# TomClabault/SYCL-ray-tracing

Measured on AMD Instinct MI355X. Metric: Msamples/sec (W×H×spp/s) at 1080p; per-channel L∞ vs CPU ref, higher is better.
Workload: dtype f32; 1 GPU; cfg2: PBRT Dragon stand-in (1,000,002 tris) 1920x1080x64spp x8 bounces, SKY-L 2048x1024 env IS+MIS; W=1920, H=1080, spp=64, bounces=8, parallelism=1 GPU

## Files before the change

sycl-ray-tracing_amd/csrc/rt_render.hip:

```cpp
#include <hip/hip_runtime.h>

#include "rt_backend_hip.h"
#include "rt_wave.h"
#include "rt_wave_kernels.h"
#include "rt_quad.h"
#include "rt_row.h"
#include "rt_octet.h"

namespace {

#if RT_DEBUG_FB
__device__ unsigned long long rt_dbg_fb[8];
#define RT_DBG(i) atomicAdd(&rt_dbg_fb[i], 1ull)
#else
#define RT_DBG(i) ((void)0)
#endif
__device__ __forceinline__ int lane_id() { return __lane_id(); }

template <int N>
struct LdsStack {
    static constexpr int CAP = N;
    uint32_t* r;
    float* k;
    __device__ __forceinline__ uint32_t rec(int i) const { return r[i * 256]; }
    __device__ __forceinline__ float key(int i) const { return k[i * 256]; }
    __device__ __forceinline__ void set(int i, uint32_t rv, float kv)
    {
        r[i * 256] = rv;
        k[i * 256] = kv;
    }
    __device__ __forceinline__ void set_rec(int i, uint32_t rv) { r[i * 256] = rv; }
};

__device__ __forceinline__ int wave_gid() { return (int)((blockIdx.x * blockDim.x + threadIdx.x) >> 6); }
__device__ __forceinline__ int wave_count() { return (int)((gridDim.x * blockDim.x) >> 6); }

template <bool STATS>
__device__ __forceinline__ void flush_stats(const rtk::Stats& st, unsigned long long* out)
{
    if (STATS)
        for (int i = 0; i < RT_STAT_COUNT; i++)
            if (st.c[i]) atomicAdd(&out[i], st.c[i]);
}

__host__ __device__ __forceinline__ size_t qbase(bool heavy, int shard, size_t seg_cap)
{
    return heavy ? ((size_t)RT_QSHARDS + (size_t)shard * (RT_QSHARDS / RT_HSHARDS)) * seg_cap : (size_t)shard * seg_cap;
}

template <class E>
__device__ __forceinline__ void append_emit(const rtk::WaveView& W, int pout, int base, int n_in, int p, const E& e)
{
    const int cps = ((n_in + 63) / 64 + RT_QSHARDS - 1) / RT_QSHARDS;
    const int sh = min(RT_QSHARDS - 1, (base >> 6) / cps);
    const size_t seg = (size_t)sh * W.seg_cap;
    const unsigned long long lt = (lane_id() == 0) ? 0ull : (~0ull >> (64 - lane_id()));
    if (W.r_heavy) {
        const int hs = sh % RT_HSHARDS;
        unsigned long long b[2 * rtk::RK_COUNT + 1];
#pragma unroll
        for (int k = 0; k < rtk::RK_COUNT; k++) {
            const bool m = (e.mask >> k) & 1u;
            b[k] = __ballot(m && !e.heavy);
            b[rtk::RK_COUNT + k] = __ballot(m && e.heavy);
        }
        b[2 * rtk::RK_COUNT] = __ballot(e.active);
        int r[2 * rtk::RK_COUNT + 1];
        if (lane_id() == 0) {
#pragma unroll
            for (int k = 0; k <= 2 * rtk::RK_COUNT; k++) {
                const int c = k < rtk::RK_COUNT ? qc_at(pout, k, sh)
                              : k < 2 * rtk::RK_COUNT ? hc_at(pout, k - rtk::RK_COUNT, hs)
                                                      : ac_at(pout, sh);
                r[k] = b[k] ? atomicAdd(W.counters + c, __popcll(b[k])) : 0;
            }
        }
#pragma unroll
        for (int k = 0; k < rtk::RK_COUNT; k++) {
            const int ih = __shfl(r[rtk::RK_COUNT + k], 0) + __popcll(b[rtk::RK_COUNT + k] & lt);
            const int i = __shfl(r[k], 0) + __popcll(b[k] & lt);
            if ((e.mask >> k) & 1u) W.q[k][e.heavy ? qbase(true, hs, W.seg_cap) + ih : qbase(false, sh, W.seg_cap) + i] = e.rec(k, p);
        }
        const int a = __shfl(r[2 * rtk::RK_COUNT], 0) + __popcll(b[2 * rtk::RK_COUNT] & lt);
        if (e.active) W.act_out[seg + a] = p;
        return;
    }
    unsigned long long b[rtk::RK_COUNT + 1];
#pragma unroll
    for (int k = 0; k < rtk::RK_COUNT; k++) b[k] = __ballot((e.mask >> k) & 1u);
    b[rtk::RK_COUNT] = __ballot(e.active);
    int r[rtk::RK_COUNT + 1];
    if (lane_id() == 0) {
#pragma unroll
        for (int k = 0; k <= rtk::RK_COUNT; k++)
            r[k] = b[k] ? atomicAdd(W.counters + (k < rtk::RK_COUNT ? qc_at(pout, k, sh) : ac_at(pout, sh)),
                                    __popcll(b[k]))
                        : 0;
    }
#pragma unroll
    for (int k = 0; k < rtk::RK_COUNT; k++) {
        const int i = __shfl(r[k], 0) + __popcll(b[k] & lt);
        if ((e.mask >> k) & 1u) W.q[k][qbase(false, sh, W.seg_cap) + i] = e.rec(k, p);
    }
    const int a = __shfl(r[rtk::RK_COUNT], 0) + __popcll(b[rtk::RK_COUNT] & lt);
    if (e.active) W.act_out[seg + a] = p;
}


template <class AT>
__device__ __forceinline__ void shard_prefix(const int32_t* cnt, int m, AT at, int* pre)
{
    const int nw = (int)(blockDim.x >> 6), w = (int)(threadIdx.x >> 6);
    for (int g = w; g < m / 64; g += nw) {
        int v = cnt[at(g * 64 + lane_id())];
        for (int o = 1; o < 64; o <<= 1) {
            const int u = __shfl_up(v, o);
            if (lane_id() >= o) v += u;
        }
        pre[g * 64 + lane_id() + 1] = v;
    }
    __syncthreads();
    int add[8];
    const int ng = m / 64;
    for (int g = w; g < ng && g < 8 * nw; g += nw) {
        int off = 0;
        for (int h = 0; h < g; h++) off += pre[h * 64 + 64];
        add[g / nw] = off;
    }
    __syncthreads();
    for (int g = w; g < ng && g < 8 * nw; g += nw) pre[g * 64 + lane_id() + 1] += add[g / nw];
    if (threadIdx.x == 0) pre[0] = 0;
    __syncthreads();
}

template <int M>
__device__ __forceinline__ int shard_find8(const int* pre, int g)
{
    constexpr int TOP = M > 512 ? 512 : M > 64 ? 64 : M > 8 ? 8 : 1;
    static_assert(M <= 4096, "three or four 8-way rounds");
    int lo = 0;
#pragma unroll
    for (int step = TOP; step >= 1; step >>= 3) {
        int c = 0;
#pragma unroll
        for (int k = 1; k < 8; k++) {
            const int j = lo + step * k;
            c += (j < M && pre[j] <= g) ? 1 : 0;
        }
        lo += step * c;
    }
    return lo;
}

__device__ __forceinline__ const rtk::RayRec* queue_item_ptr(const rtk::WaveView& W, const int* pre, int g, int& kind)
{
    const int j = shard_find8<RT_NSEG>(pre, g);
    const SegId s = seg_id(j);
    kind = s.kind;
    rtk::RayRec* qk = W.q[0];
#pragma unroll
    for (int k2 = 1; k2 < rtk::RK_COUNT; k2++) qk = s.kind == k2 ? W.q[k2] : qk;
    return qk + qbase(s.heavy, s.shard, W.seg_cap) + (g - pre[j]);
}

struct QPrefetch {
    float4_* buf;
    int* kind;
};
__device__ __forceinline__ void queue_prefetch(const rtk::WaveView& W, const int* pre, const QPrefetch& pf, int first, int cursor,
                                               int wg, int wn, int total)
{
    const int lane = lane_id(), i = lane >> 1;
    const int j = cursor + i;
    const int idx = (wg + (j >> 4) * wn) * 16 + (j & 15);
    const bool ok = lane < 32 && idx < total;
    int kind = -1;
    if (ok) {
        const rtk::RayRec* rp = queue_item_ptr(W, pre, first + idx, kind);
        __builtin_amdgcn_global_load_lds((const void*)((const float4_*)rp + (lane & 1)),
                                         (__attribute__((address_space(3))) void*)pf.buf, 16, 0, 0);
    }
    if (lane < 32 && (lane & 1) == 0) pf.kind[i] = ok ? kind : -1;
}

__global__ __launch_bounds__(256) void k_init(rtk::WaveView W)
{
    rtlibm::lds_tables_init();
    const int p = blockIdx.x * blockDim.x + threadIdx.x;
    rtk::Emit e;
    e.mask = 0;
    e.active = false;
    e.heavy = false;
    if (p < W.n_slots) rtk::path_init(W, p, e);
    append_emit(W, 0, p & ~63, W.n_slots, p, e);
}

__global__ __launch_bounds__(256) void k_resume(rtk::WaveView W)
{
    rtlibm::lds_tables_init();
    const int p = blockIdx.x * blockDim.x + threadIdx.x;
    rtk::Emit e;
    e.mask = 0;
    e.active = false;
    e.heavy = false;
    if (p < W.n_slots) rtk::path_resume(W, p, e);
    append_emit(W, 0, p & ~63, W.n_slots, p, e);
}

__global__ __launch_bounds__(256) void k_resolve(const float4_* __restrict__ base, const float4_* __restrict__ state,
                                                 float4_* __restrict__ out, int n, int done)
{
    rtlibm::lds_tables_init();
    const int i = blockIdx.x * blockDim.x + threadIdx.x;
    if (i < n) out[i] = rtk::resolve_pixel(base[i], state[i], done);
}

__global__ __launch_bounds__(256) void k_tonemap(rtk::WaveView W)
{
    rtlibm::lds_tables_init();
    const int p = blockIdx.x * blockDim.x + threadIdx.x;
    if (p < W.n_slots) rtk::tonemap_pixel(W, p);
}

#define RT_LDS_WORDS 16
#define RT_REFILL 16
#ifndef RT_TRACE_REFILL
#define RT_TRACE_REFILL 4
#endif

__device__ __forceinline__ bool forced_fallback(const rtk::WaveView& W, const float4_& o, const float4_& d)
{
    return (W.far_check && rtk::far_origin(W.S, rtk::v3of(o))) || rtk::forced_fallback(W.force_fb, o, d);
}

__device__ __forceinline__ int split_blocks(int nb, int w0, int w1)
{
    if (w0 + w1 == 0) return 0;
    int n0 = (int)((long)nb * w0 / ((long)w0 + w1));
    if (w0 > 0 && n0 == 0) n0 = 1;
    if (w1 > 0 && n0 == nb) n0 = nb - 1;
    return n0;
}

__device__ __forceinline__ void walk_done(const rtk::WaveView& W, int par, uint32_t target)
{
    const int j = atomicAdd(W.counters + C_DONE0 + par, 1);
    W.done[par][j] = (int32_t)(target >> 3);
}

template <bool ANY>
__device__ void exact_octets(const rtk::WaveView& W, int par, uint32_t* lds, int lane, int n_res, int total,
                             rtk::Stats* st)
{
    rtk::OctRing w = rtk::oct_ring(lds);
    const int sub = lane_id() & 7;
    uint32_t* spr = W.spill_r + (size_t)(lane & ~7) * RT_STACK_CAP;
    float* spk = W.spill_k + (size_t)(lane & ~7) * RT_STACK_CAP;
    const rtk::RayRec* fb = ANY ? W.fb_a[par] : W.fb_c[par];
    int32_t* ticket = W.counters + (ANY ? C_TK_EXACT_A : C_TK_EXACT_C);
    int32_t* parked = W.counters + (ANY ? C_PARKA0 : C_PARKC0) + par;
    rtk::TravG T;
    bool has = false, drained = false;
    uint32_t target = 0;
    auto done = [&]() {
        if (sub == 0) {
            if (ANY)
                rtk::finish_any(W, target, T.hit);
            else
                rtk::finish_closest(W, target, T.o, T.d, T.best_t, T.best_k);
            walk_done(W, par, target);
        }
    };
    for (;;) {
        const unsigned long long bneed = __ballot(!has && sub == 0);
        const int nneed = __popcll(bneed);
        if (!drained && (nneed >= RT_REFILL / 8 || nneed == 8)) {
            int base = 0;
            if (lane_id() == 0) base = atomicAdd(ticket, nneed);
            base = __shfl(base, 0);
            if (base + nneed >= total) drained = true;
            if (!has) {
                const int idx = base + __popcll(bneed & ((1ull << rtk::oct_lane0()) - 1ull));
                if (idx < n_res) {
                    target = ANY ? rtk::octa_resume(W.S, &W.park_a[par ^ 1][idx], T, w, sub)
                                 : rtk::octc_resume(W.S, &W.park_c[par ^ 1][idx], T, w, sub);
                    has = true;
                } else if (idx < total) {
                    const rtk::RayRec r = fb[idx - n_res];
                    target = (rt_asuint(r.o.w) << 3) | rt_asuint(r.d.w);
                    if (st && sub == 0) st->c[RT_STAT_FALLBACK]++;
                    has = rtk::octg_setup(W.S, T, rtk::v3of(r.o), rtk::v3of(r.d), st, ANY, sub);
                    if (!has) done();
                }
            }
        }
        if (!__any(has)) {
            if (drained) break;
            continue;
        }
        if (has) {
            if (ANY)
                rtk::octa_node(W.S, T, w, spr, sub, st);
            else
                rtk::octc_node(W.S, T, w, spr, spk, sub, st);
            if (T.mode == rtk::TM_DONE) {
                done();
                has = false;
            } else if (T.steps >= W.budget && (ANY ? rtk::octa_parkable(T) : rtk::octc_parkable(T))) {
                int ps = 0;
                if (sub == 0) ps = atomicAdd(parked, 1);
                if (sub == 0) RT_DBG(1);
                ps = __shfl(ps, rtk::oct_lane0());
                if (ps < W.park_cap) {
                    if (ANY)
                        rtk::octa_park(T, w, target, &W.park_a[par][ps], sub);
                    else
                        rtk::octc_park(T, w, target, &W.park_c[par][ps], sub);
                    has = false;
                } else {
                    T.steps = 0;
                }
            }
        }
    }
}

template <bool STATS, bool PROG = false>
__global__ __launch_bounds__(256) __attribute__((amdgpu_waves_per_eu(RT_STEP_OCC, 8))) void k_step(rtk::WaveView W, int par, unsigned long long* stats)
{
    __shared__ uint32_t s_lds[6 * rtk::RK_COUNT * 256];
    static_assert(6 * rtk::RK_COUNT >= RT_LDS_WORDS, "the exact roles' stacks fit the emit columns");
    __shared__ int s_pre[RT_QSHARDS + 1];
    rtlibm::lds_tables_init();
    rtk::lds_shade_init(W.S);
    int32_t* cnt = W.counters;
    if (blockIdx.x == 0 && threadIdx.x == 0) {
        cnt[C_FBC0 + (par ^ 1)] = cnt[C_FBA0 + (par ^ 1)] = 0;
        cnt[C_DONE0 + (par ^ 1)] = 0;
        const int nf = cnt[C_FBC0 + par] + cnt[C_FBA0 + par];
        if (W.handovers && nf > 0) atomicAdd(W.handovers, (unsigned long long)nf);
    }
    rtk::Stats st;
    if (STATS)
        for (int i = 0; i < RT_STAT_COUNT; i++) st.c[i] = 0;
    rtk::Stats* ps = STATS ? &st : nullptr;
    const int nrc = min(cnt[C_PARKC0 + (par ^ 1)], W.park_cap), nra = min(cnt[C_PARKA0 + (par ^ 1)], W.park_cap);
    const int ec = nrc + cnt[C_FBC0 + par], ea = nra + cnt[C_FBA0 + par];
    const int half = min(W.spill_lanes / 512, max(1, (int)gridDim.x / 4));
    constexpr int WPB = 32;
    const int nbe_c = min(half, (ec + WPB - 1) / WPB), nbe_a = min(half, (ea + WPB - 1) / WPB);
    const int b = (int)blockIdx.x;
    if (b < nbe_c) {
        exact_octets<false>(W, par, s_lds, b * 256 + (int)threadIdx.x, nrc, ec, ps);
        flush_stats<STATS>(st, stats);
        return;
    }
    if (b < nbe_c + nbe_a) {
        exact_octets<true>(W, par, s_lds, (W.spill_lanes / 512 + b - nbe_c) * 256 + (int)threadIdx.x, nra, ea, ps);
        flush_stats<STATS>(st, stats);
        return;
    }
    shard_prefix(cnt, RT_QSHARDS, [&](int j) { return ac_at(par, j); }, s_pre);
    const int n = s_pre[RT_QSHARDS];
    if (STATS && W.iterq && b == nbe_c + nbe_a && threadIdx.x == 0 && W.iter < RT_MAX_TIMED_ITERS)
        W.iterq[2 * W.iter + 1] = n;
    const int nbs = (int)gridDim.x - (nbe_c + nbe_a);
    const int wg = (b - nbe_c - nbe_a) * (int)(blockDim.x >> 6) + (int)(threadIdx.x >> 6);
    const int wn = nbs * (int)(blockDim.x >> 6);
    for (int base = wg * 64; base < n; base += wn * 64) {
        const int idx = base + lane_id();
        rtk::EmitLds<256> e;
        e.s = reinterpret_cast<float*>(s_lds) + threadIdx.x;
        e.mask = 0;
        e.active = false;
        e.heavy = false;
        int p = -1;
        if (idx < n) {
            const int sh = shard_find8<RT_QSHARDS>(s_pre, idx);
            p = W.act_in[(size_t)sh * W.seg_cap + (idx - s_pre[sh])];
            rtk::path_step<PROG>(W, p, e, ps);
        }
        append_emit(W, par ^ 1, base, n, p, e);
    }
    flush_stats<STATS>(st, stats);
}

__global__ __launch_bounds__(256) void k_hand(rtk::WaveView W, int par)
{
    __shared__ int s_pre[RT_QSHARDS + 1];
    shard_prefix(W.counters, RT_QSHARDS, [&](int j) { return ac_at(par, j); }, s_pre);
    const int n = s_pre[RT_QSHARDS];
    for (int idx = (int)(blockIdx.x * blockDim.x + threadIdx.x); idx < n; idx += (int)(gridDim.x * blockDim.x)) {
        const int sh = shard_find8<RT_QSHARDS>(s_pre, idx);
        const int p = W.act_in[(size_t)sh * W.seg_cap + (idx - s_pre[sh])];
        if ((int)rt_asuint(W.p_thr[p].w) > W.fast_thr || W.r_park[p] != 0) continue;
        const int j = atomicAdd(W.fast_ticket, 1);
        if (j >= W.fast_cap) continue;
        W.fast_list[j] = p;
        W.r_park[p] = -1;
    }
}

__global__ __launch_bounds__(256) void k_hist(rtk::WaveView W, int par, int32_t* __restrict__ hist)
{
    __shared__ int s_pre[RT_QSHARDS + 1];
    shard_prefix(W.counters, RT_QSHARDS, [&](int j) { return ac_at(par, j); }, s_pre);
    const int n = s_pre[RT_QSHARDS];
    for (int idx = (int)(blockIdx.x * blockDim.x + threadIdx.x); idx < n; idx += (int)(gridDim.x * blockDim.x)) {
        const int sh = shard_find8<RT_QSHARDS>(s_pre, idx);
        const int p = W.act_in[(size_t)sh * W.seg_cap + (idx - s_pre[sh])];
        atomicAdd(hist + min((int)rt_asuint(W.p_thr[p].w), W.spp), 1);
    }
}

__device__ __noinline__ void walk_log(const rtk::WaveView& W, rtk::V3 o, rtk::V3 d, uint32_t target, int calls, float t,
                                      int k, int where)
{
    if (W.wlog_every < 0 && t != -2.0f) return;
    if (W.wlog_every > 1 && ((target * 2654435761u) ^ ((uint32_t)W.iter * 40503u)) % (uint32_t)W.wlog_every != 0u) return;
    const int i = atomicAdd(W.wlog_n, 1);
    if (i >= W.wlog_cap) return;
    float4_* r = W.wlog + 3 * (size_t)i;
    r[0] = float4_{o.x, o.y, o.z, rt_asfloat((target & 7u) | ((uint32_t)where << 8))};
    r[1] = float4_{d.x, d.y, d.z, rt_asfloat((uint32_t)calls)};
    r[2] = float4_{t, rt_asfloat((uint32_t)k), rt_asfloat((uint32_t)W.iter), rt_asfloat(target >> 3)};
}

struct RowInQuadStack {
    static constexpr int CAP = 4 * RT_QSTACK;
    uint32_t* r;
    float* k;
    __device__ __forceinline__ uint32_t rec(int i) const { return r[(i >> 2) * 64 + (i & 3)]; }
    __device__ __forceinline__ float key(int i) const { return k[(i >> 2) * 64 + (i & 3)]; }
    __device__ __forceinline__ void set(int i, uint32_t rv, float kv)
    {
        r[(i >> 2) * 64 + (i & 3)] = rv;
        k[(i >> 2) * 64 + (i & 3)] = kv;
    }
    __device__ __forceinline__ void set_rec(int i, uint32_t rv) { r[(i >> 2) * 64 + (i & 3)] = rv; }
};

#if RT_DRAIN_STRONG_FENCE
#define RT_DRAIN_FENCE()                                       \
    do {                                                       \
        __builtin_amdgcn_fence(__ATOMIC_SEQ_CST, "workgroup"); \
        __builtin_amdgcn_s_waitcnt(0);                         \
        __builtin_amdgcn_wave_barrier();                       \
    } while (0)
#else
#define RT_DRAIN_FENCE()                                       \
    do {                                                       \
        __builtin_amdgcn_fence(__ATOMIC_ACQ_REL, "wavefront"); \
        __builtin_amdgcn_wave_barrier();                       \
    } while (0)
#endif

template <bool ANY, bool STATS, bool PAIR, int G, int BRUTE, class QSTK>
__device__ __forceinline__ void trace_stream(const rtk::WaveView& W, const RtSceneView& S, QSTK& stk, const int* s_pre,
                                             int first, int total, int wg, int wn, int32_t* fbn, rtk::RayRec* fbl,
                                             rtk::Stats* ps, const QPrefetch& pf)
{
    static_assert(G == 4 || G == 16, "quads or rows");
    constexpr int REFILL = G == 4 ? RT_TRACE_REFILL : 1;
    const int lane = lane_id(), qd = lane / G;
    int sub = lane & (G - 1);
    int cursor = 0;
    bool exhausted = wg * 16 >= total;
    bool active = false;
    uint32_t target = 0;
    rtk::QState q;
    if (!exhausted) queue_prefetch(W, s_pre, pf, first, cursor, wg, wn, total);
    auto finish = [&](int res, int gs) {
        if (W.r_heavy && sub == 0 && q.calls >= W.heavy_calls) W.r_heavy[target >> 3] = 1;
        if (STATS && W.iterq && sub == 0 && W.iter < RT_MAX_TIMED_ITERS) {
            int32_t* q2 = W.iterq + 2 * RT_MAX_TIMED_ITERS + 4 * W.iter;
            atomicMax(q2 + (ANY ? 1 : 0), q.calls);
            if (q.calls > 8) atomicAdd(q2 + 2, 1);
        }
        float t = 0.0f;
        int k = 0;
        int why = res < 0 ? 3 : 0;
        if (res > 0 && !ANY && !rtk::quad_closest_answer<BRUTE>(S, q, sub & 3, t, k, gs == 4 || sub == 0 ? ps : nullptr)) {
            res = -1;
            why = q.h.tie ? 1 : 2;
        }
        if (STATS && W.wlog && sub == 0 && q.calls >= W.wlog_min)
            walk_log(W, q.o, q.d, target, q.calls, res <= 0 ? -2.0f : ANY ? (float)(q.h.k == 1) : t, res <= 0 ? why : k,
                     gs == 4 ? 0 : 1);
        if (sub == 0) {
            if (res > 0) {
                if (ANY)
                    rtk::finish_any(W, target, q.h.k == 1);
                else
                    rtk::finish_closest(W, target, q.o, q.d, t, k);
            } else {
                fbl[atomicAdd(fbn, 1)] = rtk::RayRec{rtk::f4(q.o, rt_asfloat(target >> 3)),
                                                     rtk::f4(q.d, rt_asfloat(target & 7u))};
                RT_DBG(ANY ? 2 : 0);
                RT_DBG(why == 3 ? 3 : why == 1 ? 4 : 5);
                if (gs == 16) RT_DBG(6);
                atomicAdd(&W.r_park[target >> 3], 1);
                if (STATS && W.iterq && W.iter < RT_MAX_TIMED_ITERS)
                    atomicAdd(W.iterq + 2 * RT_MAX_TIMED_ITERS + 4 * W.iter + 3, 1);
            }
        }
    };
    constexpr int NGROUPS = 64 / G;
    static_assert(REFILL <= NGROUPS, "all groups idle triggers a refill");
    const int trig_done = NGROUPS - (G == 4 && W.drain_rows > 0 ? min(W.drain_rows, NGROUPS) : 0);
    int trig = exhausted ? trig_done : REFILL;
    for (;;) {
        const unsigned long long bidle = __ballot(!active && sub == 0);
        if (__popcll(bidle) >= trig) {
            if (!exhausted) {
                if (!active) {
                    const int j = cursor + __popcll(bidle & ((1ull << (qd * G)) - 1ull));
                    const int idx = (wg + (j >> 4) * wn) * 16 + (j & 15);
                    if (idx < total) {
                        const int slot = j - cursor;
                        __builtin_amdgcn_s_waitcnt(0x0F70);
                        rtk::RayRec r;
                        r.o = pf.buf[2 * slot];
                        r.d = pf.buf[2 * slot + 1];
                        const int kind = pf.kind[slot];
                        target = (rt_asuint(r.o.w) << 3) | (uint32_t)kind;
                        if (forced_fallback(W, r.o, r.d)) {
                            if (sub == 0) {
                                r.d.w = rt_asfloat(target & 7u);
                                fbl[atomicAdd(fbn, 1)] = r;
                                atomicAdd(&W.r_park[target >> 3], 1);
                            }
                        } else if (rtk::qstate_begin<ANY>(q, rtk::v3of(r.o), rtk::v3of(r.d), sub, ps)) {
                            active = true;
                            q.calls = 0;
                        } else if (sub == 0) {
                            if (ANY)
                                rtk::finish_any(W, target, false);
                            else
                                rtk::finish_closest(W, target, q.o, q.d, -1.0f, -1);
                        }
                    }
                }
                cursor += __popcll(bidle);
                exhausted = (wg + (cursor >> 4) * wn) * 16 >= total;
                __builtin_amdgcn_fence(__ATOMIC_ACQ_REL, "wavefront");
                __builtin_amdgcn_wave_barrier();
                if (!exhausted) queue_prefetch(W, s_pre, pf, first, cursor, wg, wn, total);
                if (STATS && lane == 0) ps->c[RT_STAT_REFILLS]++;
                trig = exhausted ? trig_done : REFILL;
            }
            const unsigned long long bact = __ballot(active && sub == 0);
            if (!bact) {
                if (exhausted) break;
                continue;
            }
            if (G == 4 && W.drain_rows > 0 && exhausted && __popcll(bact) <= W.drain_rows) break;
        }
        if (STATS) {
            if (active && sub == 0) ps->c[exhausted ? RT_STAT_DRAIN_VISITS : RT_STAT_QUAD_VISITS]++;
            if (lane == 0) ps->c[exhausted ? RT_STAT_DRAIN_SLOTS : RT_STAT_WAVE_SLOTS] += 64 / G;
        }
        if (active) {
            int res;
            if constexpr (G == 4)
                res = rtk::quad_visit<ANY, RT_VISIT_DESCEND, PAIR, BRUTE>(S, q, stk, sub, ps);
            else
                res = rtk::row_visit<ANY, RT_VISIT_DESCEND, BRUTE>(S, q, stk, sub, ps);
            q.calls += G == 4 ? 1 : 2;
            if (res != 0) {
                active = false;
                finish(res, G);
            }
        }
    }
    if constexpr (G == 4) {
        const unsigned long long bact = __ballot(active && sub == 0);
        if (!bact) return;
        const int row = lane >> 4;
        unsigned long long m = bact;
        for (int i = 0; i < row; i++) m &= m - 1ull;
#ifndef RT_DRAIN_SRC_LANE
#define RT_DRAIN_SRC_LANE 0
#endif
        const int src = (m ? __ffsll((long long)m) - 1 : 0) + RT_DRAIN_SRC_LANE;
        const bool ract = m != 0;
        auto pf = [&](float v) { return __shfl(v, src); };
        auto pi = [&](int v) { return __shfl(v, src); };
        q.o = rtk::v3(pf(q.o.x), pf(q.o.y), pf(q.o.z));
        q.d = rtk::v3(pf(q.d.x), pf(q.d.y), pf(q.d.z));
        for (int i = 0; i < 3; i++) q.rb.inv[i] = pf(q.rb.inv[i]), q.rb.oi[i] = pf(q.rb.oi[i]);
        q.h.t = pf(q.h.t), q.h.t2 = pf(q.h.t2), q.h.k = pi(q.h.k), q.h.leaf = pi(q.h.leaf);
        if (BRUTE != RT_BRUTE_OFF) q.h.prim = pi(q.h.prim);
        q.h.tie = pi(q.h.tie ? 1 : 0) != 0;
        q.sp = pi(q.sp), q.cur = pi(q.cur), q.calls = pi(q.calls);
        target = (uint32_t)pi((int)target);
        sub = lane & 15;
        const int wq = (int)(threadIdx.x >> 6) * 16;
        uint32_t* qr = stk.r - (threadIdx.x >> 2) + wq;
        float* qk = stk.k - (threadIdx.x >> 2) + wq;
        const int sq = src >> 2;
        uint32_t r0 = 0, r1 = 0;
        float k0 = 0.0f, k1 = 0.0f;
        if (ract && sub < q.sp) r0 = qr[sub * 64 + sq], k0 = qk[sub * 64 + sq];
        if (ract && sub + 16 < q.sp) r1 = qr[(sub + 16) * 64 + sq], k1 = qk[(sub + 16) * 64 + sq];
        RT_DRAIN_FENCE();
        RowInQuadStack rs{qr + 4 * row, qk + 4 * row};
        if (ract && sub < q.sp) rs.set(sub, r0, k0);
        if (ract && sub + 16 < q.sp) rs.set(sub + 16, r1, k1);
        RT_DRAIN_FENCE();
        active = ract;
#if RT_DRAIN_RESTART == 1
        q.sp = 0;
        if (q.cur != rtk::RT_CUR_NONE) q.cur = 0;
#elif RT_DRAIN_RESTART == 2
        if (ract) rtk::qstate_begin<ANY>(q, q.o, q.d, sub, nullptr);
#elif RT_DRAIN_RESTART == 3
        q.rb = rtk::rayb_setup(q.o, q.d);
#elif RT_DRAIN_RESTART == 4
        q.h.t = __builtin_inff(), q.h.t2 = __builtin_inff(), q.h.k = ANY ? 0 : -1, q.h.leaf = -1;
        q.h.prim = 0x7fffffff, q.h.tie = false, q.h.ovf = false;
        q.sp = 0;
        if (q.cur != rtk::RT_CUR_NONE) q.cur = 0;
#endif
        while (__any(active)) {
            if (STATS) {
                if (active && sub == 0) ps->c[RT_STAT_DRAIN_VISITS]++;
                if (lane == 0) ps->c[RT_STAT_DRAIN_SLOTS] += 4;
            }
            if (active) {
                const int res = rtk::row_visit<ANY, RT_VISIT_DESCEND, BRUTE>(S, q, rs, sub, ps);
                q.calls += 2;
                if (res != 0) {
                    active = false;
                    finish(res, 16);
                }
            }
        }
    }
}

template <bool STATS, bool PAIR = true, int G = 4, int BRUTE = RT_BRUTE_SCENE>
__global__ __launch_bounds__(256) __attribute__((amdgpu_waves_per_eu(RT_TRACE_OCC, 8))) void k_trace(rtk::WaveView W, int par, unsigned long long* stats)
{
    __shared__ uint32_t s_lds[RT_LDS_WORDS * 256];
    __shared__ int s_pre[RT_NSEG + 1];
    __shared__ float4_ s_qbuf[4][64];
    __shared__ int s_qkind[4][16];
    const QPrefetch pf{s_qbuf[threadIdx.x >> 6], s_qkind[threadIdx.x >> 6]};
    int32_t* cnt = W.counters;
    if (blockIdx.x == 0) {
        for (int j = threadIdx.x; j < (rtk::RK_COUNT + 1) * RT_QSHARDS; j += blockDim.x)
            cnt[j < rtk::RK_COUNT * RT_QSHARDS ? qc_at(par ^ 1, j / RT_QSHARDS, j % RT_QSHARDS)
                                                : ac_at(par ^ 1, j - rtk::RK_COUNT * RT_QSHARDS)] = 0;
        for (int j = threadIdx.x; j < rtk::RK_COUNT * RT_HSHARDS; j += blockDim.x)
            cnt[hc_at(par ^ 1, j / RT_HSHARDS, j % RT_HSHARDS)] = 0;
        if (threadIdx.x == 0) {
            cnt[C_PARKC0 + par] = cnt[C_PARKA0 + par] = 0;
            cnt[C_TK_EXACT_C] = cnt[C_TK_EXACT_A] = 0;
        }
    }
    {
        const int nd = cnt[C_DONE0 + (par ^ 1)];
        for (int j = (int)(blockIdx.x * blockDim.x + threadIdx.x); j < nd; j += (int)(gridDim.x * blockDim.x))
            atomicSub(&W.r_park[W.done[par ^ 1][j]], 1);
    }
    rtk::Stats st;
    if (STATS)
        for (int i = 0; i < RT_STAT_COUNT; i++) st.c[i] = 0;
    rtk::Stats* ps = STATS ? &st : nullptr;
    const int b = (int)blockIdx.x;

    const RtSceneView S = W.S;
    shard_prefix(cnt, RT_NSEG, [&](int j) { return seg_counter(par, j); }, s_pre);
    const int c0 = 0, a0 = s_pre[RT_SEG_AH];
    const int nc = (W.any_rays ? a0 : s_pre[RT_SEG_END]) - c0;
    const int na = W.any_rays ? s_pre[RT_SEG_END] - a0 : 0;
    if (STATS && W.iterq && b == 0 && threadIdx.x == 0 && W.iter < RT_MAX_TIMED_ITERS) W.iterq[2 * W.iter] = nc + na;
    const int fb0 = 0, nbf = (int)gridDim.x;
    const int nbc = split_blocks(nbf, nc, na);
    const bool closest = b - fb0 < nbc;
    const int rb = closest ? b - fb0 : b - fb0 - nbc;
    const int rnb = closest ? nbc : nbf - nbc;
    const int wg = rb * (int)(blockDim.x >> 6) + (int)(threadIdx.x >> 6);
    const int wn = rnb * (int)(blockDim.x >> 6);
    const int total = closest ? nc : na;
    int32_t* fbn = cnt + (closest ? C_FBC0 : C_FBA0) + par;
    rtk::RayRec* fbl = closest ? W.fb_c[par] : W.fb_a[par];
    if constexpr (G == 4) {
        rtk::QuadStack<RT_QSTACK, 64> stk{s_lds + (threadIdx.x >> 2), (float*)s_lds + RT_QSTACK * 64 + (threadIdx.x >> 2)};
        if (closest)
            trace_stream<false, STATS, PAIR, 4, BRUTE>(W, S, stk, s_pre, c0, total, wg, wn, fbn, fbl, ps, pf);
        else
            trace_stream<true, STATS, PAIR, 4, BRUTE>(W, S, stk, s_pre, a0, total, wg, wn, fbn, fbl, ps, pf);
    } else {
        static_assert(2 * RT_RSTACK * 16 <= RT_LDS_WORDS * 256, "row stacks fit k_trace's LDS");
        rtk::QuadStack<RT_RSTACK, 16> stk{s_lds + (threadIdx.x >> 4), (float*)s_lds + RT_RSTACK * 16 + (threadIdx.x >> 4)};
        if (closest)
            trace_stream<false, STATS, PAIR, 16, BRUTE>(W, S, stk, s_pre, c0, total, wg, wn, fbn, fbl, ps, pf);
        else
            trace_stream<true, STATS, PAIR, 16, BRUTE>(W, S, stk, s_pre, a0, total, wg, wn, fbn, fbl, ps, pf);
    }
    flush_stats<STATS>(st, stats);
}

using TailEmit = rtk::EmitLds<RT_TAIL_MAXP>;
__device__ __forceinline__ void tail_lists(const TailEmit& e, int last_kind, uint8_t* l0, uint8_t* l1, int* nl)
{
    const int lane = lane_id();
    nl[0] = nl[1] = 0;
#pragma unroll
    for (int k = 0; k < rtk::RK_COUNT; k++) {
        const bool want = (e.mask >> k) & 1u;
        const unsigned long long b = __ballot(want);
        const int l = k <= last_kind ? 0 : 1;
        if (want) (l ? l1 : l0)[nl[l] + __popcll(b & ((1ull << lane) - 1ull))] = (uint8_t)((lane << 3) | k);
        nl[l] += __popcll(b);
    }
}
__device__ __noinline__ int tail_step(const rtk::WaveView& W, int my, int last_kind, float* cols, uint8_t* l0, uint8_t* l1,
                                      rtk::Stats* ps)
{
    TailEmit e;
    e.s = cols + (lane_id() & (RT_TAIL_MAXP - 1));
    e.mask = 0;
    e.active = false;
    e.heavy = false;
    if (my >= 0) rtk::path_step<true>(W, my, e, ps);
    int nl[2];
    tail_lists(e, last_kind, l0, l1, nl);
    return (e.active ? 1 : 0) | (nl[0] << 1) | (nl[1] << 11);
}
template <class XS>
__device__ __noinline__ void tail_exact(const rtk::WaveView& W, int l, uint32_t target, rtk::V3 o, rtk::V3 d, XS& xs,
                                        rtk::Stats* ps)
{
    if (l == 0) {
        rtk::TravC T;
        if (rtk::travc_begin(W.S, T, o, d, ps))
            while (rtk::travc_step(W.S, T, xs, ps)) {
            }
        rtk::finish_closest(W, target, T.o, T.d, T.best_t, T.best_k);
    } else {
        rtk::TravA T;
        if (rtk::trava_begin(W.S, T, o, d, ps))
            while (rtk::trava_step(W.S, T, xs, ps)) {
            }
        rtk::finish_any(W, target, T.hit);
    }
}
#ifndef RT_TAIL_DESCEND
#define RT_TAIL_DESCEND RT_VISIT_DESCEND
#endif
template <bool STATS, bool PAIR, int G, bool FAST>
__device__ __forceinline__ void tail_body(const rtk::WaveView& W, int par, unsigned long long* stats, int blk)
{
    __shared__ float s_em[4][6 * rtk::RK_COUNT * RT_TAIL_MAXP];
    __shared__ uint8_t s_q[4][2][RT_TAIL_MAXP * rtk::RK_COUNT];
    __shared__ int s_my[4][RT_TAIL_MAXP];
    __shared__ uint32_t s_stk[2 * RT_QSTACK * 64];
    __shared__ int s_pre[RT_QSHARDS + 1];
    rtlibm::lds_tables_init();
    rtk::lds_shade_init(W.S);
    int32_t* cnt = W.counters;
    shard_prefix(cnt, RT_QSHARDS, [&](int j) { return ac_at(par, j); }, s_pre);
    const int n = FAST ? min(s_pre[RT_QSHARDS], W.fast_cap) : s_pre[RT_QSHARDS];
    const RtSceneView S = W.S;
    rtk::Stats st;
    if (STATS)
        for (int i = 0; i < RT_STAT_COUNT; i++) st.c[i] = 0;
    rtk::Stats* ps = STATS ? &st : nullptr;
    static_assert(G == 4 || G == 16, "quads or rows");
    constexpr int SCAP = G == 4 ? RT_QSTACK : RT_RSTACK, GPB = 256 / G;
    static_assert(2 * SCAP * GPB <= 2 * RT_QSTACK * 64, "group stacks fit k_tail's LDS");
    const int wv = (int)(threadIdx.x >> 6), lane = lane_id(), sub = lane & (G - 1), qd = (int)(threadIdx.x / G);
    using STK = rtk::QuadStack<SCAP, GPB>;
    STK stk{s_stk + qd, (float*)s_stk + SCAP * GPB + qd};
    const size_t gl = (size_t)blk * blockDim.x + threadIdx.x;
    rtk::SpillStack<STK> xs{stk, W.spill_r + gl * RT_STACK_CAP, W.spill_k + gl * RT_STACK_CAP};
    const int P = W.tail_paths;
    const int last_kind = W.any_rays ? rtk::RK_CAM : rtk::RK_BENV;
    int my = -1;
    bool drained = false;
    int rounds = 0;
    long long tk_step = 0, tk_walk = 0;
    long long tk_solo = 0;
    int trips = 0, solo_trips = 0;
    const bool probe = STATS && W.iterq && W.iter + 1 < RT_MAX_TIMED_ITERS;
    for (;;) {
        const bool need = lane < P && my < 0;
        const unsigned long long bneed = __ballot(need);
        if (bneed && !drained) {
            const int nneed = __popcll(bneed);
            int base = 0;
            if (lane == 0) base = atomicAdd(cnt + C_TK_TAIL, nneed);
            base = __shfl(base, 0);
            if (base + nneed >= n) drained = true;
            const int idx = base + __popcll(bneed & ((1ull << lane) - 1ull));
            if (need && idx < n) {
                const int sh = shard_find8<RT_QSHARDS>(s_pre, idx);
                my = W.act_in[(size_t)sh * W.seg_cap + (idx - s_pre[sh])];
                if (FAST) W.r_park[my] = 0;
            }
        }
        if (!__any(my >= 0)) break;
        rounds++;
        const long long t0 = probe ? wall_clock64() : 0;
        int nl[2];
        {
            if (lane < RT_TAIL_MAXP) s_my[wv][lane] = my;
            const int r = tail_step(W, my, last_kind, s_em[wv], s_q[wv][0], s_q[wv][1], ps);
            if (!(r & 1)) my = -1;
            nl[0] = (r >> 1) & 0x3ff;
            nl[1] = r >> 11;
        }
        long long t1 = 0;
        if (probe) {
            t1 = wall_clock64();
            tk_step += __shfl(t1, 0) - __shfl(t0, 0);
        }
        __builtin_amdgcn_fence(__ATOMIC_RELEASE, "wavefront");
        __builtin_amdgcn_wave_barrier();
        const int nq = nl[0] + nl[1];
        int next = 0;
        bool act = false;
        int l = 0;
        uint32_t target = 0;
        rtk::QState q;
        for (;;) {
            bool exact = false;
            const unsigned long long bidle = __ballot(!act && sub == 0);
            if (next < nq) {
                const int qi = next + __popcll(bidle & ((1ull << (lane & ~(G - 1))) - 1ull));
                if (!act && qi < nq) {
                    l = qi < nl[0] ? 0 : 1;
                    const int ent = s_q[wv][l][l ? qi - nl[0] : qi], j = ent >> 3, kind = ent & 7;
                    TailEmit ce;
                    ce.s = s_em[wv] + j;
                    rtk::RayRec r;
                    r.o = rtk::f4(ce.o(kind), 0.0f);
                    r.d = rtk::f4(ce.d(kind), 0.0f);
                    target = ((uint32_t)s_my[wv][j] << 3) | (uint32_t)kind;
                    q.o = rtk::v3of(r.o);
                    q.d = rtk::v3of(r.d);
                    if (forced_fallback(W, r.o, r.d)) {
                        exact = true;
                    } else {
                        act = l ? rtk::qstate_begin<true>(q, q.o, q.d, sub, ps) : rtk::qstate_begin<false>(q, q.o, q.d, sub, ps);
                        if (STATS) q.calls = 0;
                        if (!act && sub == 0) {
                            if (l == 0)
                                rtk::finish_closest(W, target, q.o, q.d, -1.0f, -1);
                            else
                                rtk::finish_any(W, target, false);
// ... 144 lines not shown
```

sycl-ray-tracing_amd/csrc/rt_wave_layout.h:

```cpp
#pragma once

#include <hip/hip_runtime.h>

#include "rt_wave.h"

#ifndef RT_DEBUG_FB
#define RT_DEBUG_FB 0
#endif

#ifndef RT_STEP_OCC
#define RT_STEP_OCC 3
#endif
#ifndef RT_STEP_FILL
#define RT_STEP_FILL RT_STEP_OCC
#endif
#ifndef RT_TAIL_ROWS
#define RT_TAIL_ROWS 1
#endif
#ifndef RT_HEAVY_CALLS
#define RT_HEAVY_CALLS 6
#endif
#ifndef RT_TRACE_OCC
#define RT_TRACE_OCC 6
#endif
#ifndef RT_DRAIN_ROWS
#define RT_DRAIN_ROWS 3
#endif
#define RT_TAIL_MAXP 16
#ifndef RT_TAIL_OCC
#define RT_TAIL_OCC 3
#endif
#define RT_QSTACK 32
#define RT_RSTACK 64

enum {
    C_FBC0 = 0,
    C_FBC1,
    C_FBA0,
    C_FBA1,
    C_PARKC0,
    C_PARKC1,
    C_PARKA0,
    C_PARKA1,
    C_TK_EXACT_C,
    C_TK_EXACT_A,
    C_TK_TAIL,
    C_DONE0,
    C_DONE1,
    C_SHARDED = 64,
};
#define RT_QSHARDS 64
#define RT_HSHARDS 8
#define RT_CSTRIDE 32
#define C_HEAVY (C_SHARDED + (2 * rtk::RK_COUNT + 2) * RT_QSHARDS * RT_CSTRIDE)
#define C_COUNT (C_HEAVY + 2 * rtk::RK_COUNT * RT_HSHARDS * RT_CSTRIDE)
#define C_ZERO (C_SHARDED - 1)
__host__ __device__ __forceinline__ int qc_at(int par, int kind, int shard)
{
    return C_SHARDED + ((par * rtk::RK_COUNT + kind) * RT_QSHARDS + shard) * RT_CSTRIDE;
}
__host__ __device__ __forceinline__ int ac_at(int par, int shard)
{
    return C_SHARDED + ((2 * rtk::RK_COUNT + par) * RT_QSHARDS + shard) * RT_CSTRIDE;
}
__host__ __device__ __forceinline__ int hc_at(int par, int kind, int shard)
{
    return C_HEAVY + ((par * rtk::RK_COUNT + kind) * RT_HSHARDS + shard) * RT_CSTRIDE;
}

#define RT_NCK 4
#define RT_SEG_CH (RT_NCK * RT_HSHARDS)
#define RT_SEG_AH (RT_SEG_CH + RT_NCK * RT_QSHARDS)
#define RT_SEG_A (RT_SEG_AH + (rtk::RK_COUNT - RT_NCK) * RT_HSHARDS)
#define RT_SEG_END (RT_SEG_A + (rtk::RK_COUNT - RT_NCK) * RT_QSHARDS)
#define RT_NSEG ((RT_SEG_END + 63) / 64 * 64)
struct SegId {
    int kind, shard;
    bool heavy;
};
__host__ __device__ __forceinline__ SegId seg_id(int j)
{
    SegId s;
    if (j < RT_SEG_CH) {
        s.heavy = true, s.kind = j / RT_HSHARDS, s.shard = j % RT_HSHARDS;
    } else if (j < RT_SEG_AH) {
        s.heavy = false, s.kind = (j - RT_SEG_CH) / RT_QSHARDS, s.shard = (j - RT_SEG_CH) % RT_QSHARDS;
    } else if (j < RT_SEG_A) {
        s.heavy = true, s.kind = RT_NCK + (j - RT_SEG_AH) / RT_HSHARDS, s.shard = (j - RT_SEG_AH) % RT_HSHARDS;
    } else {
        s.heavy = false, s.kind = RT_NCK + (j - RT_SEG_A) / RT_QSHARDS, s.shard = (j - RT_SEG_A) % RT_QSHARDS;
    }
    return s;
}
__host__ __device__ __forceinline__ int seg_counter(int par, int j)
{
    if (j >= RT_SEG_END) return C_ZERO;
    const SegId s = seg_id(j);
    return s.heavy ? hc_at(par, s.kind, s.shard) : qc_at(par, s.kind, s.shard);
}
```

sycl-ray-tracing_amd/csrc/rt_wave_run.hip:

```cpp
#include <hip/hip_runtime.h>

#include <cstdio>
#include <string>
#include <vector>
#include <algorithm>

#include <chrono>
#include <thread>

#include "rt_backend_hip.h"
#include "rt_wave.h"
#include "rt_wave_kernels.h"

size_t rt_wave_counter_bytes() { return C_COUNT * sizeof(int32_t); }
size_t rt_wave_readback_bytes() { return RT_QSHARDS * RT_CSTRIDE * 4 + 64; }

namespace {
const int threads = rt_wave_threads;
const WaveKnobs knobs{RT_TRACE_OCC, RT_TAIL_OCC, RT_HEAVY_CALLS, RT_TAIL_ROWS, RT_DRAIN_ROWS, RT_TAIL_MAXP, RT_QSHARDS};

enum class Await { None, Live, Fallbacks };
enum class Fast { Waiting, HistPending, HandNext, Handed, NoShare };

struct WaveLane {
    rtk::WaveView W{};
    int32_t* lists[2] = {nullptr, nullptr};
    int32_t* cnt = nullptr;
    int32_t* h = nullptr;
    hipStream_t s = nullptr;
    hipEvent_t ev = nullptr;
    int n = 0, it = 0, tail_iter = -1;
    long live = 0;
    bool done = false, tail_next = false;
    Await await = Await::None;
    Fast fast = Fast::NoShare;
    int fast_thr = 0, fast_n = 0;
    Event (*tev)[RT_MAX_TIMED_ITERS] = nullptr;
};

struct WaveRun {
    rt_context* c;
    Backend* b;
    int w, h, spp, bounces;
    const rtk::PixSrc& src;
    int n;
    float4_* fb;
    hipStream_t s;
    const WavePass* pass;
    bool linear;
    int dev_cus = 256;
    WavePlan P{};
    WaveLane L[RT_MAX_LANES];
    bool S = false, SEQ = false, wlog = false;
    unsigned long long* stats = nullptr;
    const char* iter_log = nullptr;
    hipStream_t fstream = nullptr;
    bool fast_launched = false, fast_ran = false;
    long max_iters = 0;
    static constexpr size_t act_bytes = RT_QSHARDS * RT_CSTRIDE * 4;

    int begin();
    int init_lane(int l);
    int launch_trace(WaveLane& La);
    int fast_launch();
    int fast_threshold(WaveLane& La);
    int launch_step(WaveLane& La);
    int launch_tail(WaveLane& La, int par);
    int read_live(WaveLane& La);
    int issue(WaveLane& La);
    int process(WaveLane& La);
    int start_hist(WaveLane& La);
    int poll();
    int finish();
    int report();
    int lane_of(const WaveLane& La) const { return (int)(&La - L); }
    int step_blocks_of(const WaveLane& La) const
    {
        return (int)std::max(3l, std::min((La.live + threads - 1) / threads, (long)dev_cus * RT_STEP_FILL));
    }
    int trace_blocks_of(const WaveLane& La) const
    {
        const long want = (20 * La.live + 2 * threads - 1) / (2 * threads);
        return (int)std::min((long)P.trace_blocks, std::max(want, (long)dev_cus * 4 + 64));
    }
};

int WaveRun::begin()
{
    if (int r = b->ev_done.wait(c, s)) return r;
    (void)hipDeviceGetAttribute(&dev_cus, hipDeviceAttributeMultiprocessorCount, b->device);
    const RtDiag& dg = c->diag;
    S = c->stats_enabled;
    SEQ = S && c->stats_seq;
    stats = (unsigned long long*)b->stats.p;
    if (S) HIPCHK(c, hipMemsetAsync(b->stats.p, 0, b->stats.bytes, s));
    iter_log = dg.iter_log.empty() ? nullptr : dg.iter_log.c_str();
    wlog = S && dg.wlog_cap > 0 && b->index == 0;
    if (wlog) {
        if (int r = ensure(c, b->wlog, 256 + (size_t)dg.wlog_cap * 48)) return r;
        HIPCHK(c, hipMemsetAsync(b->wlog.p, 0, 256, s));
    }
    if (!b->handovers.p) {
        if (int r = ensure(c, b->handovers, 8)) return r;
        HIPCHK(c, hipMemsetAsync(b->handovers.p, 0, 8, s));
    }
    if (S && iter_log) {
        if (int r = ensure(c, b->iterq, RT_MAX_TIMED_ITERS * 24)) return r;
        HIPCHK(c, hipMemsetAsync(b->iterq.p, 0, RT_MAX_TIMED_ITERS * 24, s));
    }
    const int rows = src.xy ? 0 : n / src.W;
    P = wave_plan(c->sched, knobs, WaveSource{src.xy != nullptr, src.W, src.off, src.stride}, n, rows, spp, dev_cus, SEQ,
                  b->lanes, b->budget);
    const int nl = P.lanes;
    if (P.fast_k > 0 && nl == RT_MAX_LANES && !b->fs) HIPCHK(c, hipStreamCreateWithFlags(&b->fs.h, hipStreamNonBlocking));
    fstream = P.fast_k > 0 ? (hipStream_t)(nl < RT_MAX_LANES ? b->ls[nl] : b->fs) : nullptr;
    if (nl > 1) {
        HIPCHK(c, hipEventRecord(b->ev_fork, s));
        for (int l = 1; l < nl; l++) HIPCHK(c, hipStreamWaitEvent(b->ls[l], b->ev_fork, 0));
    }
    for (int l = 0; l < nl; l++)
        if (int r = init_lane(l)) return r;
    if (dg.verbose)
        fprintf(stderr, "[rt] run_wave n=%d lanes=%d cus=%d trace_blocks=%d budget=%d\n", n, nl, dev_cus, P.trace_blocks,
                L[0].W.budget);
    max_iters = 64l * spp * ((long)bounces + 1) + 4096;
    for (int l = 0; l < nl; l++)
        if (int r = issue(L[l])) return r;
    return RT_OK;
}

int WaveRun::init_lane(int l)
{
    WaveLane& La = L[l];
    const LanePlan& lp = P.lane[l];
    const RtDiag& dg = c->diag;
    rtk::PixSrc ls = src;
    if (src.xy) ls.xy = src.xy + 2 * (size_t)lp.first;
    ls.off = lp.off;
    ls.stride = lp.stride;
    La.n = lp.n;
    La.live = La.n;
    La.s = l == 0 ? s : (hipStream_t)b->ls[l];
    La.cnt = (int32_t*)b->counters[l].p;
    La.h = b->h_act[l];
    La.ev = b->ev_lane[l];
    La.tev = b->tev[l];
    rtk::WaveView& W = La.W;
    W.park_cap = 1 << 16;
    W.heavy_calls = P.heavy_calls;
    W.spec_cam = P.spec_cam;
    W.shards = RT_QSHARDS;
    W.seg_cap = lp.seg_cap;
    W.spill_lanes = dev_cus * 4 * threads;
    W.fspill_lanes = 0;
    const size_t need = rtk::wave_carve(nullptr, (size_t)La.n, W);
    if (int r = ensure(c, b->wave[l], need)) return r;
    rtk::wave_carve((char*)b->wave[l].p, (size_t)La.n, W);
    W.S = b->view;
    rt_view_near(c, W.S);
    W.cam = c->cam;
    W.src = ls;
    W.W = w;
    W.H = h;
    W.spp = spp;
    W.bounces = bounces;
    W.prog = pass ? pass->state + lp.first : nullptr;
    W.first = pass ? pass->first : 0;
    W.seed_spp = pass ? pass->seed_spp : spp;
// ... 410 lines not shown
```

Before: 1104 Msamples/s.

## Replace static trace chunk striding with sharded atomic ticket work stealing

Trace waves used to walk a fixed strided sequence of 16-ray chunks. They now draw chunks from 16 sharded atomic ticket counters, prefetching the next chunk early. After finishing their own stream (closest or any-hit), waves also process the other stream. This is meant to balance load when ray traversal costs are uneven, at the cost of one atomic per chunk and some extra code paths.

```diff
diff --git a/sycl-ray-tracing_amd/csrc/rt_render.hip b/sycl-ray-tracing_amd/csrc/rt_render.hip
--- a/sycl-ray-tracing_amd/csrc/rt_render.hip
+++ b/sycl-ray-tracing_amd/csrc/rt_render.hip
@@ -167,12 +167,31 @@
     float4_* buf;
     int* kind;
 };
-__device__ __forceinline__ void queue_prefetch(const rtk::WaveView& W, const int* pre, const QPrefetch& pf, int first, int cursor,
-                                               int wg, int wn, int total)
-{
+struct ChunkSrc {
+    int32_t* ticket;
+    int shard;
+    int wg, wn;
+};
+__device__ __forceinline__ int next_chunk(const ChunkSrc& cs, int prev)
+{
+#if RT_TRACE_STATIC
+    return prev < 0 ? cs.wg : prev + cs.wn;
+#else
+    int t = 0;
+    if (lane_id() == 0) t = atomicAdd(cs.ticket, 1);
+    return __builtin_amdgcn_readfirstlane(t) * RT_TK_SHARDS + cs.shard;
+#endif
+}
+struct ChunkCursor {
+    int cur, next, off;
+    __device__ __forceinline__ int idx(int j) const { return (j < 16 ? cur : next) * 16 + (j & 15); }
+};
+__device__ __forceinline__ void queue_prefetch(const rtk::WaveView& W, const int* pre, const QPrefetch& pf, int first,
+                                               ChunkCursor& cc, const ChunkSrc& cs, int total)
+{
+    if (cc.off > 0 && cc.next < 0) cc.next = next_chunk(cs, cc.cur);
     const int lane = lane_id(), i = lane >> 1;
-    const int j = cursor + i;
-    const int idx = (wg + (j >> 4) * wn) * 16 + (j & 15);
+    const int idx = cc.idx(cc.off + i);
     const bool ok = lane < 32 && idx < total;
     int kind = -1;
     if (ok) {
@@ -334,6 +353,7 @@
     rtlibm::lds_tables_init();
     rtk::lds_shade_init(W.S);
     int32_t* cnt = W.counters;
+    if (!RT_TRACE_STATIC && blockIdx.x == 0 && threadIdx.x < 2 * RT_TK_SHARDS) cnt[C_TK_TRACE_C + threadIdx.x * RT_CSTRIDE] = 0;
     if (blockIdx.x == 0 && threadIdx.x == 0) {
         cnt[C_FBC0 + (par ^ 1)] = cnt[C_FBA0 + (par ^ 1)] = 0;
         cnt[C_DONE0 + (par ^ 1)] = 0;
@@ -457,19 +477,23 @@
 
 template <bool ANY, bool STATS, bool PAIR, int G, int BRUTE, class QSTK>
 __device__ __forceinline__ void trace_stream(const rtk::WaveView& W, const RtSceneView& S, QSTK& stk, const int* s_pre,
-                                             int first, int total, int wg, int wn, int32_t* fbn, rtk::RayRec* fbl,
+                                             int first, int total, const ChunkSrc& cs, int32_t* fbn, rtk::RayRec* fbl,
                                              rtk::Stats* ps, const QPrefetch& pf)
 {
     static_assert(G == 4 || G == 16, "quads or rows");
     constexpr int REFILL = G == 4 ? RT_TRACE_REFILL : 1;
     const int lane = lane_id(), qd = lane / G;
     int sub = lane & (G - 1);
-    int cursor = 0;
-    bool exhausted = wg * 16 >= total;
+    ChunkCursor cc{0, -1, 0};
+    bool exhausted = (RT_TRACE_STATIC ? cs.wg : cs.shard) * 16 >= total;
+    if (!exhausted) {
+        cc.cur = next_chunk(cs, -1);
+        exhausted = cc.cur * 16 >= total;
+    }
     bool active = false;
     uint32_t target = 0;
     rtk::QState q;
-    if (!exhausted) queue_prefetch(W, s_pre, pf, first, cursor, wg, wn, total);
+    if (!exhausted) queue_prefetch(W, s_pre, pf, first, cc, cs, total);
     auto finish = [&](int res, int gs) {
         if (W.r_heavy && sub == 0 && q.calls >= W.heavy_calls) W.r_heavy[target >> 3] = 1;
         if (STATS && W.iterq && sub == 0 && W.iter < RT_MAX_TIMED_ITERS) {
@@ -514,10 +538,8 @@
         if (__popcll(bidle) >= trig) {
             if (!exhausted) {
                 if (!active) {
-                    const int j = cursor + __popcll(bidle & ((1ull << (qd * G)) - 1ull));
-                    const int idx = (wg + (j >> 4) * wn) * 16 + (j & 15);
-                    if (idx < total) {
-                        const int slot = j - cursor;
+                    const int slot = __popcll(bidle & ((1ull << (qd * G)) - 1ull));
+                    if ((unsigned)cc.idx(cc.off + slot) < (unsigned)total) {
                         __builtin_amdgcn_s_waitcnt(0x0F70);
                         rtk::RayRec r;
                         r.o = pf.buf[2 * slot];
@@ -541,11 +563,16 @@
                         }
                     }
                 }
-                cursor += __popcll(bidle);
-                exhausted = (wg + (cursor >> 4) * wn) * 16 >= total;
+                cc.off += __popcll(bidle);
+                if (cc.off >= 16) {
+                    cc.off -= 16;
+                    cc.cur = cc.next >= 0 ? cc.next : next_chunk(cs, cc.cur);
+                    cc.next = -1;
+                }
+                exhausted = cc.cur * 16 + cc.off >= total;
                 __builtin_amdgcn_fence(__ATOMIC_ACQ_REL, "wavefront");
                 __builtin_amdgcn_wave_barrier();
-                if (!exhausted) queue_prefetch(W, s_pre, pf, first, cursor, wg, wn, total);
+                if (!exhausted) queue_prefetch(W, s_pre, pf, first, cc, cs, total);
                 if (STATS && lane == 0) ps->c[RT_STAT_REFILLS]++;
                 trig = exhausted ? trig_done : REFILL;
             }
@@ -683,22 +710,29 @@
     const int rnb = closest ? nbc : nbf - nbc;
     const int wg = rb * (int)(blockDim.x >> 6) + (int)(threadIdx.x >> 6);
     const int wn = rnb * (int)(blockDim.x >> 6);
-    const int total = closest ? nc : na;
-    int32_t* fbn = cnt + (closest ? C_FBC0 : C_FBA0) + par;
-    rtk::RayRec* fbl = closest ? W.fb_c[par] : W.fb_a[par];
-    if constexpr (G == 4) {
-        rtk::QuadStack<RT_QSTACK, 64> stk{s_lds + (threadIdx.x >> 2), (float*)s_lds + RT_QSTACK * 64 + (threadIdx.x >> 2)};
-        if (closest)
-            trace_stream<false, STATS, PAIR, 4, BRUTE>(W, S, stk, s_pre, c0, total, wg, wn, fbn, fbl, ps, pf);
-        else
-            trace_stream<true, STATS, PAIR, 4, BRUTE>(W, S, stk, s_pre, a0, total, wg, wn, fbn, fbl, ps, pf);
-    } else {
-        static_assert(2 * RT_RSTACK * 16 <= RT_LDS_WORDS * 256, "row stacks fit k_trace's LDS");
-        rtk::QuadStack<RT_RSTACK, 16> stk{s_lds + (threadIdx.x >> 4), (float*)s_lds + RT_RSTACK * 16 + (threadIdx.x >> 4)};
-        if (closest)
-            trace_stream<false, STATS, PAIR, 16, BRUTE>(W, S, stk, s_pre, c0, total, wg, wn, fbn, fbl, ps, pf);
-        else
-            trace_stream<true, STATS, PAIR, 16, BRUTE>(W, S, stk, s_pre, a0, total, wg, wn, fbn, fbl, ps, pf);
+    const int shard = (b * (int)(blockDim.x >> 6) + (int)(threadIdx.x >> 6)) % RT_TK_SHARDS;
+#pragma clang loop unroll(disable)
+    for (int turn = 0; turn < (RT_TRACE_STATIC ? 1 : 2); turn++) {
+        const bool cl = closest == (turn == 0);
+        const int total = cl ? nc : na;
+        if (total == 0) continue;
+        const ChunkSrc cs{cnt + (cl ? C_TK_TRACE_C : C_TK_TRACE_A) + shard * RT_CSTRIDE, shard, wg, wn};
+        int32_t* fbn = cnt + (cl ? C_FBC0 : C_FBA0) + par;
+        rtk::RayRec* fbl = cl ? W.fb_c[par] : W.fb_a[par];
+        if constexpr (G == 4) {
+            rtk::QuadStack<RT_QSTACK, 64> stk{s_lds + (threadIdx.x >> 2), (float*)s_lds + RT_QSTACK * 64 + (threadIdx.x >> 2)};
+            if (cl)
+                trace_stream<false, STATS, PAIR, 4, BRUTE>(W, S, stk, s_pre, c0, total, cs, fbn, fbl, ps, pf);
+            else
+                trace_stream<true, STATS, PAIR, 4, BRUTE>(W, S, stk, s_pre, a0, total, cs, fbn, fbl, ps, pf);
+        } else {
+            static_assert(2 * RT_RSTACK * 16 <= RT_LDS_WORDS * 256, "row stacks fit k_trace's LDS");
+            rtk::QuadStack<RT_RSTACK, 16> stk{s_lds + (threadIdx.x >> 4), (float*)s_lds + RT_RSTACK * 16 + (threadIdx.x >> 4)};
+            if (cl)
+                trace_stream<false, STATS, PAIR, 16, BRUTE>(W, S, stk, s_pre, c0, total, cs, fbn, fbl, ps, pf);
+            else
+                trace_stream<true, STATS, PAIR, 16, BRUTE>(W, S, stk, s_pre, a0, total, cs, fbn, fbl, ps, pf);
+        }
     }
     flush_stats<STATS>(st, stats);
 }
diff --git a/sycl-ray-tracing_amd/csrc/rt_wave_layout.h b/sycl-ray-tracing_amd/csrc/rt_wave_layout.h
--- a/sycl-ray-tracing_amd/csrc/rt_wave_layout.h
+++ b/sycl-ray-tracing_amd/csrc/rt_wave_layout.h
@@ -53,7 +53,15 @@
 #define RT_HSHARDS 8
 #define RT_CSTRIDE 32
 #define C_HEAVY (C_SHARDED + (2 * rtk::RK_COUNT + 2) * RT_QSHARDS * RT_CSTRIDE)
-#define C_COUNT (C_HEAVY + 2 * rtk::RK_COUNT * RT_HSHARDS * RT_CSTRIDE)
+#ifndef RT_TK_SHARDS
+#define RT_TK_SHARDS 16
+#endif
+#define C_TK_TRACE_C (C_HEAVY + 2 * rtk::RK_COUNT * RT_HSHARDS * RT_CSTRIDE)
+#define C_TK_TRACE_A (C_TK_TRACE_C + RT_TK_SHARDS * RT_CSTRIDE)
+#define C_COUNT (C_TK_TRACE_A + RT_TK_SHARDS * RT_CSTRIDE)
+#ifndef RT_TRACE_STATIC
+#define RT_TRACE_STATIC 0
+#endif
 #define C_ZERO (C_SHARDED - 1)
 __host__ __device__ __forceinline__ int qc_at(int par, int kind, int shard)
 {
diff --git a/sycl-ray-tracing_amd/csrc/rt_wave_run.hip b/sycl-ray-tracing_amd/csrc/rt_wave_run.hip
--- a/sycl-ray-tracing_amd/csrc/rt_wave_run.hip
+++ b/sycl-ray-tracing_amd/csrc/rt_wave_run.hip
@@ -14,6 +14,14 @@
 
 size_t rt_wave_counter_bytes() { return C_COUNT * sizeof(int32_t); }
 size_t rt_wave_readback_bytes() { return RT_QSHARDS * RT_CSTRIDE * 4 + 64; }
+extern "C" int rt_wave_counter_layout(int* out, int n)
+{
+    const int v[] = {C_COUNT,      C_SHARDED,    C_HEAVY,    C_HEAVY + 2 * rtk::RK_COUNT * RT_HSHARDS * RT_CSTRIDE,
+                     C_TK_TRACE_C, C_TK_TRACE_A, RT_TK_SHARDS, RT_CSTRIDE, RT_TRACE_STATIC};
+    const int m = (int)(sizeof v / sizeof v[0]);
+    for (int i = 0; i < m && i < n; i++) out[i] = v[i];
+    return m;
+}
 
 namespace {
 const int threads = rt_wave_threads;
```

After: 1068 Msamples/s. -3.3%, worse.
